# adobe-research/DiffusionHandles

Hardware: AMD Instinct MI355X
Metric: guided-denoise steps/sec at 512x512 (SD2-depth) (higher is better)
Workload: dtype f16; 1 GPU; single 512x512 edit per GPU, SD2-depth (865.9M params, seeded random weights), guided phase: 3 x (fwd + energy + bwd-to-latent) + CFG fwd (B=2) + DDIM step; resolution=512, edits_per_gpu=1, correspondences=24906, parallelism=independent edits, one process per GPU, no collectives

## Files before the change

### diffusionhandles_amd/_lib.py

```python
import ctypes
import os

import torch

_HERE = os.path.dirname(os.path.abspath(__file__))
LIB_PATH = os.environ.get("DIFFHANDLES_LIB") or os.path.join(_HERE, "libdiffhandles_hip.so")
_LIB = None

c_p = ctypes.c_void_p
c_i = ctypes.c_int
c_f = ctypes.c_float
c_d = ctypes.c_double
c_sz = ctypes.c_size_t


class UNetConfig(ctypes.Structure):
    _fields_ = [("in_channels", c_i), ("out_channels", c_i), ("n_levels", c_i),
                ("block_out_channels", c_i * 4), ("layers_per_block", c_i), ("heads", c_i * 4),
                ("cross_attention_dim", c_i), ("norm_groups", c_i), ("sample_size", c_i),
                ("text_len", c_i), ("max_batch", c_i), ("dtype", c_i), ("max_diff_batch", c_i)]


class VAEConfig(ctypes.Structure):
    _fields_ = [("latent_channels", c_i), ("out_channels", c_i), ("block_out_channels", c_i * 4),
# ... 88 lines not shown
    "dh_latent_update": (c_i, [c_p, c_p, c_p, c_f, c_f, c_i, c_p]),
    "dh_adam_step": (c_i, [c_p, c_p, c_p, c_p, c_f, c_f, c_f, c_f, c_i, c_i, c_p]),
    "dh_mse_fwd_bwd": (c_i, [c_p, c_p, c_i, c_p, c_p, c_p]),
    "dh_latent_update_strided": (c_i, [c_p, c_p, c_p, c_i, c_i, c_f, c_f, c_i, c_p]),
    "dh_pack_sample": (c_i, [c_p, c_p, c_i, c_i, c_p, c_i, c_i, c_i, c_i, c_p]),
    "dh_unet_io_ptr": (c_i, [c_p, c_i, c_i, ctypes.POINTER(c_p), ctypes.POINTER(c_sz)]),
    "dh_mse_cotangent": (c_i, [c_p, c_p, c_i, c_f, c_f, c_p, c_p, c_p, c_p]),
    "dh_adam_step_scaled": (c_i, [c_p, c_p, c_p, c_p, c_p, c_f, c_f, c_f, c_f, c_i, c_i, c_p]),
    "dh_mse_cotangent_batch": (c_i, [c_p, c_p, c_i, c_i, c_f, c_f, c_d, c_p, c_p, c_p, c_p, c_p, c_p]),
    "dh_adam_step_scaled_batch": (c_i, [c_p, c_p, c_p, c_p, c_p, c_p, c_f, c_f, c_f, c_f, c_i, c_i, c_i, c_p]),
    "dh_latent_update_guarded": (c_i, [c_p, c_p, c_p, c_i, c_i, c_f, c_i, c_i, c_p, c_i, c_i, c_p, c_p, c_i, c_i, c_p]),
    "dh_ddim_cfg_step_flagged": (c_i, [c_p, c_p, c_p, c_p, c_f, c_f, c_f, c_i, c_i, c_p, c_i, c_i, c_p]),
}

c_l = ctypes.c_long
DEBUG_SIGNATURES = {
    "dh_dbg_gemm": (c_i, [c_i, c_p, c_l, c_p, c_i, c_i, c_i, c_i, c_i, c_i, c_i, c_i, c_i, c_i, c_i, c_p, c_p, c_i, c_i,
                          c_p, c_l, c_p, c_l, c_i, c_p, c_sz, c_p]),
    "dh_dbg_gemm_groupnorm": (c_i, [c_i, c_p, c_l, c_p, c_i, c_i, c_i, c_i, c_i, c_i, c_i, c_p, c_p, c_p, c_sz, c_i, c_i, c_p, c_p, c_f, c_i,
                                    c_p, c_p, c_p, ctypes.POINTER(c_i), c_p]),
    "dh_dbg_gemm_groupnorm_bwd": (c_i, [c_i, c_p, c_l, c_p, c_i, c_i, c_i, c_i, c_i, c_i, c_i, c_p, c_p, c_sz, c_i, c_i, c_p, c_p, c_p, c_p, c_i,
                                        c_p, c_p, ctypes.POINTER(c_i), c_p]),
    "dh_dbg_gemm_groupnorm_res": (c_i, [c_i, c_p, c_l, c_p, c_i, c_i, c_i, c_i, c_i, c_i, c_i, c_p, c_p, c_l, c_p, c_p, c_sz, c_i, c_i, c_p, c_p,
                                    c_f, c_i, c_p, c_p, c_p, ctypes.POINTER(c_i), c_p]),
    "dh_dbg_gemm_groupnorm_bwd_res": (c_i, [c_i, c_p, c_l, c_p, c_i, c_i, c_i, c_i, c_i, c_i, c_i, c_p, c_l, c_p, c_p, c_sz, c_i, c_i, c_p, c_p, c_p,
                                        c_p, c_i, c_p, c_p, ctypes.POINTER(c_i), c_p]),
    "dh_dbg_concat_groupnorm": (c_i, [c_i, c_p, c_i, c_p, c_i, c_p, c_i, c_i, c_i, c_p, c_p, c_f, c_i, c_p, c_p, c_p, c_p]),
    "dh_dbg_gemm_last_tile": (c_i, [ctypes.POINTER(c_i)]),
    "dh_dbg_unet_concat_ops": (c_i, [ctypes.POINTER(UNetConfig), ctypes.POINTER(c_i), c_i, ctypes.POINTER(c_i)]),
    "dh_dbg_gemm_lnfold": (c_i, [c_i, c_p, c_l, c_p, c_i, c_i, c_i, c_p, c_p, c_p, c_f, c_p, c_l, c_p]),
    "dh_dbg_gemm_glu": (c_i, [c_i, c_i, c_p, c_l, c_p, c_i, c_i, c_i, c_p, c_p, c_p, c_p, c_p, c_p]),
    "dh_dbg_gemm_glub_split": (c_i, [c_i, c_p, c_l, c_p, c_i, c_i, c_i, c_i, c_p, c_l, c_i, c_p, c_p, ctypes.POINTER(c_i), c_p]),
    "dh_dbg_unet_ff_fold": (c_i, [c_p, c_i, ctypes.POINTER(c_i), ctypes.POINTER(c_i), c_p, c_p, c_p]),
    "dh_dbg_gemm_family": (c_i, [c_i]),
    "dh_dbg_gemm_stage": (c_i, [c_i]),
    "dh_dbg_gemm_xattn": (c_i, [c_i, c_p, c_l, c_p, c_i, c_i, c_i, c_p, c_p, c_p, c_p, c_f, c_p, c_p, c_p, c_l, c_p, c_p, c_i, c_i, c_i,
                                ctypes.POINTER(c_i), c_p]),
    "dh_dbg_gemm_xattn_dq": (c_i, [c_i, c_p, c_l, c_p, c_i, c_i, c_i, c_p, c_p, c_p, c_p, c_l, c_p, c_p, c_p, c_i, c_i, ctypes.POINTER(c_i), c_p]),
    "dh_dbg_gemm_xattn_carried": (c_i, [ctypes.POINTER(c_i), ctypes.POINTER(ctypes.c_longlong)]),
    "dh_dbg_gemm_pp_variant": (c_i, [c_i, c_p]),
    "dh_dbg_gemm_pp_ablate": (c_i, [c_i]),
    "dh_dbg_gemm_pp_persist": (c_i, [c_i]),
    "dh_dbg_gemm_pp_glu": (c_i, [c_i]),
    "dh_dbg_gemm_pp_plan": (c_i, [c_i, c_i, c_i, c_i, c_i, c_i, c_sz, ctypes.POINTER(c_i), ctypes.POINTER(c_i), ctypes.POINTER(c_i)]),
    "dh_dbg_touch_tiled": (c_i, [c_sz, c_p]),
    "dh_dbg_groupnorm": (c_i, [c_i, c_p, c_p, c_p, c_p, c_p, c_p, c_p, c_p, c_i, c_i, c_i, c_i, c_f, c_i, c_i, c_p]),
    "dh_dbg_layernorm": (c_i, [c_i, c_p, c_p, c_p, c_p, c_p, c_p, c_p, c_p, c_i, c_i, c_f, c_p]),
    "dh_dbg_geglu": (c_i, [c_i, c_p, c_p, c_p, c_p, c_i, c_i, c_p]),
    "dh_dbg_attention": (c_i, [c_i, c_p, c_l, c_p, c_p, c_l, c_p, c_l, c_p, c_p, c_p, c_p, c_p, c_p, c_i, c_i, c_i, c_i, c_p]),
    "dh_dbg_attention_bwd_pair": (c_i, [c_i, c_p, c_l, c_p, c_p, c_l, c_p, c_l, c_p, c_p, c_p, c_p, c_p, c_p, c_i, c_i, c_i, c_i, c_p, c_p]),
    "dh_dbg_pool2x2": (c_i, [c_i, c_p, c_p, c_i, c_i, c_i, c_i, c_i, c_p]),
    "dh_dbg_ellipse_offsets": (c_i, [c_i, ctypes.POINTER(ctypes.c_int32), c_i, ctypes.POINTER(c_i)]),
    "dh_dbg_lane_ops": (c_i, [c_p, c_p, c_p, c_p]),
}


def lib():
    global _LIB
    if _LIB is None:
        if not os.path.exists(LIB_PATH):
            raise RuntimeError(
                f"native HIP library not found at {LIB_PATH}; build it with "
                "`python -c 'import __graft_entry__ as g; g.build()'` (there is no CPU fallback)")
        handle = ctypes.CDLL(LIB_PATH)
        missing = []
        for name, (res, args) in list(SIGNATURES.items()) + list(DEBUG_SIGNATURES.items()):
# ... 39 lines not shown
```

### diffusionhandles_amd/csrc/unet_engine.cpp

```cpp
#include <stdlib.h>

#include <algorithm>
#include <map>
#include <numeric>
#include <vector>

#include "unet_kernels.h"

namespace dh {

enum OpType { OP_CONV_IN, OP_CONV_OUT, OP_GEMM, OP_GN, OP_LN, OP_ATTN, OP_GEGLU, OP_CONCAT, OP_TIMESTEP, OP_T2F };
enum ParamKind { PK_F32, PK_MAT };

struct Ten {
  size_t off = 0, goff = 0;
  size_t off_fo = 0;
  int rows = 0, C = 0;
  int ld = 0;
  int view = -1, col = 0;
  bool req_grad = true;
  bool persistent = false;
};

struct Wt {
  size_t fwd_off = 0, bwd_off = 0;
  int N = 0, K = 0, taps = 1;
  bool has_bwd = true, f32 = false;
  int glu_F = 0;
};

struct ParamInfo {
  std::string name;
  int ndim = 0;
  int64_t shape[4] = {0, 0, 0, 0};
  int kind = PK_F32;
  size_t f32_off = 0;
  int wt = -1;
  int row_off = 0;
  int glu_F = 0;
};

struct Op {
  int type = OP_GEMM;
// ... 15 lines not shown
  int xattn_bwd_op = -1;
};

struct FfFold {
  int wt_po = -1, wt_ffo = -1, wt = -1;
  long b_po = -1, b_ffo = -1, bias = -1;
};

}

using namespace dh;

struct dh_unet {
  dh_unet_config cfg;
  int dtype = DH_DTYPE_F16;
  std::vector<Ten> tens;
  std::vector<Wt> wts;
  std::vector<ParamInfo> params;
  std::vector<Op> ops;
  std::vector<FfFold> ffolds;
  std::map<std::string, int> pindex;
  size_t w16_elems = 0, pf_elems = 0, act_elems = 0, grad_elems = 0, f32_elems = 0;
  size_t fo_elems = 0;
  size_t partial_elems = 0, scratch_elems = 0, small_elems = 0;
  unsigned short *w16 = nullptr, *act = nullptr, *grad = nullptr, *scratch = nullptr;
  float *pf = nullptr, *f32a = nullptr, *partial = nullptr, *small = nullptr;
  int t_text = -1, t_kv = -1, t_conv_in_out = -1, t_final = -1, act_ids[3] = {-1, -1, -1};
  int act_op_end[3] = {0, 0, 0};
  int first_cross_op = 0;
  int saved_ops = 0;
  int temb_ops = 0, temb_rows = 0;
  float temb_t = 0.f;
  hipStream_t temb_stream = nullptr;
  uint64_t text_key = 0, kv_key = 0;
  int kv_rows = 0;
  hipStream_t kv_stream = nullptr;
  long temb_f32_off = -1;
  int temb_total = 0, kv_total = 0;
  float *in_sample = nullptr, *in_text = nullptr, *io_eps = nullptr, *out_dsample = nullptr, *out_dtext = nullptr, *t_dev = nullptr;
  std::map<uint64_t, hipGraphExec_t> graphs;
  std::map<uint64_t, double> graph_flops;
  bool use_graphs = true;
  long ones_off = -1, zeros_off = -1;
  bool fold_dirty = true;
  bool owns_weights = true;
  int n_shared = 0;
  int saved_batch = 0;
  const float* saved_sample = nullptr;
  std::vector<char> gready;
  double flops_fwd = 0, flops_bwd = 0;
  int64_t launches = 0;

  bool fo_mode = false;
  unsigned short* aptr(int t, int B_unused = 0) { return act + (fo_mode && !tens[t].persistent ? tens[t].off_fo : tens[t].off); }
  std::vector<int> galias;
  unsigned short* gptr(int t) {
    while (galias[t] != t) t = galias[t];
    return grad + tens[t].goff;
  }
};

namespace {

struct Builder {
  dh_unet& u;
  int maxB, maxBd;
// ... 51 lines not shown

  int gn(int x, const std::string& pre, float eps, bool silu) {
    const Ten tx = u.tens[x];
    Op o;
    o.type = OP_GN; o.in0 = x; o.out = tensor(tx.rows, tx.C);
    o.gamma_off = param_f32(pre + ".weight", tx.C);
    o.beta_off = param_f32(pre + ".bias", tx.C);
    o.eps = eps; o.silu = silu; o.groups = u.cfg.norm_groups;
    o.stats_off = f32_slot((size_t)maxB * o.groups * 2);
    u.ops.push_back(o);
    return o.out;
  }
  int ln(int x, const std::string& pre) {
    const Ten tx = u.tens[x];
    Op o;
    o.type = OP_LN; o.in0 = x; o.out = tensor(tx.rows, tx.C);
    o.gamma_off = param_f32(pre + ".weight", tx.C);
    o.beta_off = param_f32(pre + ".bias", tx.C);
    o.eps = 1e-5f;
    o.stats_off = f32_slot((size_t)maxB * tx.rows * 2);
    u.ops.push_back(o);
    return o.out;
  }
  int conv3(int x, const std::string& pre, int Cout, int Hs, int stride, int up, long temb_off, int res) {
    const Ten& tx = u.tens[x];
    const int Cin = tx.C;
    const int Hv = Hs << up, Ho = stride == 2 ? Hv / 2 : Hv;
    Op o;
    o.type = OP_GEMM; o.mode = A_CONV3; o.in0 = x; o.res = res;
    o.Hin = Hs; o.Win = Hs; o.Cin = Cin; o.Hout = Ho; o.Wout = Ho; o.stride = stride; o.up = up;
    o.wt = weight(Cout, 9 * Cin, 9);
    bind_mat(pre + ".weight", o.wt, Cout, 0, Cin, 9);
    o.bias_off = param_f32(pre + ".bias", Cout);
    if (temb_off >= 0) { o.rowvec_off = u.temb_f32_off + temb_off; o.rowvec_ld = u.temb_total; }
    o.out = tensor(Ho * Ho, Cout);
    u.ops.push_back(o);
    return o.out;
  }
  int linear_w(int x, int wt, long bias_off, int res, int in_col = 0, int in_cols = 0, bool silu = false,
               bool req_grad = true) {
    const Ten tx = u.tens[x];
    Op o;
    o.type = OP_GEMM; o.mode = A_DENSE; o.in0 = x; o.res = res; o.wt = wt; o.bias_off = bias_off;
    o.in_col = in_col; o.in_cols = in_cols ? in_cols : tx.C; o.act_silu = silu;
    o.out = tensor(tx.rows, u.wts[wt].N, req_grad);
    u.ops.push_back(o);
    return o.out;
  }
  int linear(int x, const std::string& pre, int N, bool bias, int res, bool as_conv1x1 = false) {
    const int K = u.tens[x].C;
    const int wt = weight(N, K);
    if (as_conv1x1) bind_conv1x1(pre + ".weight", wt, N, K); else bind_mat(pre + ".weight", wt, N, 0, K, 1);
    const long b = bias ? param_f32(pre + ".bias", N) : -1;
    return linear_w(x, wt, b, res);
  }
  int concat(int a, int b) {
    Op o;
    o.type = OP_CONCAT; o.in0 = a; o.in1 = b;
    o.out = tensor(u.tens[a].rows, u.tens[a].C + u.tens[b].C);
    u.ops.push_back(o);
    return o.out;
  }

  void fold_ln_into_last_gemm() {
    const int gi = (int)u.ops.size() - 1, li = gi - 1;
    Op& g = u.ops[gi];
    Op& l = u.ops[li];
// ... 96 lines not shown
  }
  temb_total += 2 * c.block_out_channels[L - 1];
  kv_total += 2 * c.block_out_channels[L - 1];
  for (int i = 0; i < L; ++i) {
    const int ch = c.block_out_channels[L - 1 - i];
    temb_total += (n + 1) * ch;
    if (i > 0) kv_total += (n + 1) * 2 * ch;
  }
}

static void layout_tensors(dh_unet& u);
static size_t ff_fold_scratch(int C);

int build(dh_unet& u) {
  const dh_unet_config& c = u.cfg;
  Builder b(u);
  const int L = c.n_levels, n = c.layers_per_block, S = c.sample_size;
  const int* ch = c.block_out_channels;
  const int temb_dim = ch[0] * 4;
  count_fused(c, u.temb_total, u.kv_total);

  int t_sin = b.tensor(1, ch[0], false);
  { Op o; o.type = OP_TIMESTEP; o.out = t_sin; u.ops.push_back(o); }
  const int w1 = b.weight(temb_dim, ch[0], 1, false);
  b.bind_mat("time_embedding.linear_1.weight", w1, temb_dim, 0, ch[0], 1);
  int e1 = b.linear_w(t_sin, w1, b.param_f32("time_embedding.linear_1.bias", temb_dim), -1, 0, 0, true, false);
  const int w2 = b.weight(temb_dim, temb_dim, 1, false);
  b.bind_mat("time_embedding.linear_2.weight", w2, temb_dim, 0, temb_dim, 1);
  int e2 = b.linear_w(e1, w2, b.param_f32("time_embedding.linear_2.bias", temb_dim), -1, 0, 0, true, false);
  b.wt_temb = b.weight(u.temb_total, temb_dim, 1, false);
  b.temb_bias_off = u.pf_elems;
  u.pf_elems += align_up((size_t)u.temb_total, 64);
  int t_temb = b.linear_w(e2, b.wt_temb, (long)b.temb_bias_off, -1, 0, 0, false, false);
  u.temb_f32_off = (long)b.f32_slot((size_t)c.max_batch * u.temb_total);
  { Op o; o.type = OP_T2F; o.in0 = t_temb; u.ops.push_back(o); }
  u.temb_ops = (int)u.ops.size();

  u.t_text = b.tensor(c.text_len, c.cross_attention_dim, true);
  b.wt_kv = b.weight(u.kv_total, c.cross_attention_dim);
  u.t_kv = b.linear_w(u.t_text, b.wt_kv, -1, -1);

  { Op o;
    o.type = OP_CONV_IN;
    o.wt = b.weight(ch[0], 9 * c.in_channels, 9, true, true);
    b.bind_mat("conv_in.weight", o.wt, ch[0], 0, c.in_channels, 9);
    o.bias_off = b.param_f32("conv_in.bias", ch[0]);
    o.Hin = S; o.Cin = c.in_channels;
    o.out = b.tensor(S * S, ch[0]);
    u.t_conv_in_out = o.out;
    u.ops.push_back(o); }
  int x = u.t_conv_in_out;
  std::vector<int> skips{x};
  int H = S;
  for (int i = 0; i < L; ++i) {
    const std::string pre = "down_blocks." + std::to_string(i);
    const bool attn = i < L - 1, down = i < L - 1;
    for (int j = 0; j < n; ++j) {
      x = b.resnet(x, pre + ".resnets." + std::to_string(j), ch[i], H);
      if (attn) x = b.transformer(x, pre + ".attentions." + std::to_string(j), c.heads[i], H);
      skips.push_back(x);
    }
    if (down) {
      x = b.conv3(x, pre + ".downsamplers.0.conv", ch[i], H, 2, 0, -1, -1);
      H /= 2;
      skips.push_back(x);
    }
  }
// ... 309 lines not shown
    dh_unet_destroy(u);
    return DH_ERR_HIP;
  };
  hipError_t e;
  if (parent) {
    if (u->w16_elems != parent->w16_elems || u->pf_elems != parent->pf_elems) {
      set_error("internal: shared engine lays its parameters out differently");
      delete u;
      return DH_ERR_STATE;
    }
    u->owns_weights = false;
    u->w16 = parent->w16; u->pf = parent->pf;
    u->fold_dirty = false;
  } else {
    if ((e = hipMalloc((void**)&u->w16, u->w16_elems * 2 + 256)) != hipSuccess) return fail(e, "hipMalloc weights");
    if ((e = hipMalloc((void**)&u->pf, u->pf_elems * 4 + 256)) != hipSuccess) return fail(e, "hipMalloc f32 params");
  }
  if ((e = hipMalloc((void**)&u->act, u->act_elems * 2 + 256)) != hipSuccess) return fail(e, "hipMalloc activations");
  if ((e = hipMalloc((void**)&u->grad, u->grad_elems * 2 + 256)) != hipSuccess) return fail(e, "hipMalloc gradients");
  if ((e = hipMalloc((void**)&u->f32a, u->f32_elems * 4 + 256)) != hipSuccess) return fail(e, "hipMalloc f32 arena");
  if ((e = hipMalloc((void**)&u->partial, u->partial_elems * 4)) != hipSuccess) return fail(e, "hipMalloc split-K");
  if ((e = hipMalloc((void**)&u->scratch, u->scratch_elems * 2)) != hipSuccess) return fail(e, "hipMalloc scratch");
  if ((e = hipMalloc((void**)&u->small, u->small_elems * 4)) != hipSuccess) return fail(e, "hipMalloc small");
  {
    const dh_unet_config& c = u->cfg;
    const size_t ns = (size_t)c.max_batch * c.sample_size * c.sample_size;
    const size_t nt = (size_t)c.max_batch * c.text_len * c.cross_attention_dim;
    if ((e = hipMalloc((void**)&u->in_sample, ns * c.in_channels * 4)) != hipSuccess) return fail(e, "hipMalloc staging");
    if ((e = hipMalloc((void**)&u->out_dsample, ns * c.in_channels * 4)) != hipSuccess) return fail(e, "hipMalloc staging");
    if ((e = hipMalloc((void**)&u->io_eps, ns * c.out_channels * 4)) != hipSuccess) return fail(e, "hipMalloc staging");
    if ((e = hipMalloc((void**)&u->in_text, nt * 4)) != hipSuccess) return fail(e, "hipMalloc staging");
    if ((e = hipMalloc((void**)&u->out_dtext, nt * 4)) != hipSuccess) return fail(e, "hipMalloc staging");
    if ((e = hipMalloc((void**)&u->t_dev, 64)) != hipSuccess) return fail(e, "hipMalloc staging");
    u->use_graphs = !(getenv("DH_GRAPH") && atoi(getenv("DH_GRAPH")) == 0);
  }
  if (!parent) {
    (void)hipMemset(u->w16, 0, u->w16_elems * 2);
    (void)hipMemset(u->pf, 0, u->pf_elems * 4);
  }
  u->gready.assign(u->tens.size(), 0);
  u->galias.resize(u->tens.size());
  std::iota(u->galias.begin(), u->galias.end(), 0);
  *out = u;
  return DH_OK;
}

extern "C" int dh_unet_create_shared(dh_unet* parent, int max_batch, void* stream, dh_unet** out) {
  DH_REQUIRE(parent && out, "null pointer");
  DH_REQUIRE(parent->owns_weights, "share from the engine that owns the weights");
  dh_unet_config cfg = parent->cfg;
  if (max_batch > 0 && max_batch != cfg.max_batch) { cfg.max_batch = max_batch; cfg.max_diff_batch = 0; }
  DH_REQUIRE(cfg.max_batch < 4096 && (long)cfg.max_batch * cfg.sample_size * cfg.sample_size < (1L << 21), "bad max_batch");
  if (parent->fold_dirty) {
    fold_layernorms(parent, (hipStream_t)stream);
    DH_CHECK_HIP(hipStreamSynchronize((hipStream_t)stream));
  }
  int rc = create_engine(&cfg, parent, out);
  if (rc == DH_OK) ++parent->n_shared;
  return rc;
}

extern "C" void dh_unet_destroy(dh_unet* u) {
  if (!u) return;
  if (u->owns_weights) { (void)hipFree(u->w16); (void)hipFree(u->pf); }
  (void)hipFree(u->act); (void)hipFree(u->grad);
  (void)hipFree(u->f32a); (void)hipFree(u->partial); (void)hipFree(u->scratch); (void)hipFree(u->small);
  (void)hipFree(u->in_sample); (void)hipFree(u->in_text); (void)hipFree(u->io_eps); (void)hipFree(u->out_dsample);
  (void)hipFree(u->out_dtext); (void)hipFree(u->t_dev);
  for (auto& kv : u->graphs) (void)hipGraphExecDestroy(kv.second);
  delete u;
}

extern "C" int dh_unet_num_params(const dh_unet* u) { return u ? (int)u->params.size() : 0; }

extern "C" int dh_unet_param_info(const dh_unet* u, int i, const char** name, int* ndim, int64_t* shape4) {
  DH_REQUIRE(u && i >= 0 && i < (int)u->params.size() && name && ndim && shape4, "bad arguments");
  const ParamInfo& p = u->params[i];
  *name = p.name.c_str();
  *ndim = p.ndim;
  for (int k = 0; k < 4; ++k) shape4[k] = p.shape[k];
  return DH_OK;
}

extern "C" int dh_unet_load_param(dh_unet* u, int i, const float* src, void* stream) {
  DH_REQUIRE(u && src && i >= 0 && i < (int)u->params.size(), "bad arguments");
  if (!u->owns_weights || u->n_shared > 0) {
    set_error("dh_unet_load_param: the weights are shared (dh_unet_create_shared): load every parameter before sharing");
    return DH_ERR_STATE;
  }
  u->temb_rows = 0; u->fold_dirty = true; u->kv_key = 0;
  hipStream_t st = (hipStream_t)stream;
  const ParamInfo& p = u->params[i];
  if (p.kind == PK_F32) {
    if (p.glu_F) {
      hipLaunchKernelGGL(k_load_glu_bias, dim3(cdiv((int)p.shape[0], 256)), dim3(256), 0, st, src, u->pf + p.f32_off, p.glu_F);
      DH_LAUNCH_CHECK();
      return DH_OK;
    }
    DH_CHECK_HIP(hipMemcpyAsync(u->pf + p.f32_off, src, (size_t)p.shape[0] * 4, hipMemcpyDeviceToDevice, st));
    return DH_OK;
  }
  const Wt& w = u->wts[p.wt];
  const int N = (int)p.shape[0], C = (int)p.shape[1], taps = w.taps;
  const size_t total = (size_t)N * C * taps;
  const unsigned nb = (unsigned)((total + 255) / 256);
  const long fwd_ld = w.K;
  const long bwd_ld = (long)taps * w.N;
  if (w.f32) {
    float* f = u->pf + w.fwd_off;
    float* b = w.has_bwd ? u->pf + w.bwd_off : nullptr;
    hipLaunchKernelGGL((k_load_weight<float, false>), dim3(nb), dim3(256), 0, st, src, N, C, taps, f, fwd_ld, (long)p.row_off,
                       b, bwd_ld, (long)p.row_off, w.N);
  } else if (u->dtype == DH_DTYPE_F16) {
    f16* f = (f16*)(u->w16 + w.fwd_off);
    f16* b = w.has_bwd ? (f16*)(u->w16 + w.bwd_off) : nullptr;
    hipLaunchKernelGGL((k_load_weight<f16, true>), dim3(nb), dim3(256), 0, st, src, N, C, taps, f, fwd_ld, (long)p.row_off, b,
                       bwd_ld, (long)p.row_off, w.N, 1.f, w.glu_F);
  } else {
    bf16* f = (bf16*)(u->w16 + w.fwd_off);
    bf16* b = w.has_bwd ? (bf16*)(u->w16 + w.bwd_off) : nullptr;
    hipLaunchKernelGGL((k_load_weight<bf16, true>), dim3(nb), dim3(256), 0, st, src, N, C, taps, f, fwd_ld, (long)p.row_off, b,
                       bwd_ld, (long)p.row_off, w.N, 1.f, w.glu_F);
  }
  DH_LAUNCH_CHECK();
  return DH_OK;
}

extern "C" size_t dh_unet_weight_bytes(const dh_unet* u) { return u && u->owns_weights ? u->w16_elems * 2 + u->pf_elems * 4 : 0; }
extern "C" size_t dh_unet_workspace_bytes(const dh_unet* u) {
  return u ? (u->act_elems + u->grad_elems + u->scratch_elems) * 2 + (u->f32_elems + u->partial_elems + u->small_elems) * 4 : 0;
}

static void fill_gemm(dh_unet* u, const Op& o, int B, GemmArgs& g) {
  const Wt& w = u->wts[o.wt];
  const Ten& ti = u->tens[o.in0];
  const Ten& to = u->tens[o.out];
  g.A = u->aptr(o.in0) + o.in_col; g.lda = ti.ld;
  g.W = u->w16 + w.fwd_off;
  g.M = B * to.rows; g.N = w.N; g.K = w.K;
  g.mode = o.mode; g.Hin = o.Hin; g.Win = o.Win; g.Cin = o.Cin; g.Hout = o.Hout; g.Wout = o.Wout;
  g.stride = o.stride; g.up = o.up;
  g.bias = o.bias_off >= 0 ? u->pf + o.bias_off : nullptr;
  if (o.rowvec_off >= 0) { g.rowvec = u->f32a + o.rowvec_off; g.rowvec_ld = o.rowvec_ld; g.rows_per_batch = to.rows; }
  if (o.res >= 0) { g.R = u->aptr(o.res); g.ldr = u->tens[o.res].ld; }
  g.C = u->aptr(o.out); g.ldc = to.ld;
  g.act_silu = o.act_silu;
  g.partial = u->partial; g.partial_elems = u->partial_elems;
  if (o.ln_fold >= 0) {
    const Op& l = u->ops[o.ln_fold];
    if (use_ln_fold(u, B)) {
      g.A = u->aptr(l.in0); g.lda = u->tens[l.in0].ld;
      g.bias = nullptr;
      g.ln_s = u->pf + o.ln_s_off; g.ln_t = u->pf + o.ln_t_off; g.ln_stats = u->f32a + l.stats_off; g.ln_eps = l.eps;
    } else {
      g.bias = u->pf + o.ln_t_off;
    }
  }
}

static void forward_ops(dh_unet* u, int B, int n_ops, int first_op, bool kv_hit, bool save, hipStream_t st) {
  const int dt = u->dtype;
  const dh_unet_config& c = u->cfg;
  u->flops_fwd = 0;
  int gn_have = 0;
  int xa_have = 0;
  if (!kv_hit) launch_f32_to_t(dt, u->in_text, u->aptr(u->t_text), (size_t)B * c.text_len * c.cross_attention_dim, st);
  for (int oi = first_op; oi < n_ops; ++oi) {
    const Op& o = u->ops[oi];
    if (kv_hit && oi == u->temb_ops) continue;
    switch (o.type) {
      case OP_TIMESTEP:
        launch_timestep_embedding(dt, u->t_dev, c.block_out_channels[0], B, u->aptr(o.out), st);
        break;
      case OP_T2F:
        launch_t_to_f32(dt, u->aptr(o.in0), u->f32a + u->temb_f32_off, (size_t)B * u->temb_total, 0, st);
        break;
      case OP_CONV_IN: {
        const Wt& w = u->wts[o.wt];
        launch_conv_small_fwd(dt, u->in_sample, 1, u->pf + w.fwd_off, u->pf + o.bias_off, u->aptr(o.out), 0, B, o.Hin, o.Hin,
                              o.Cin, w.N, st);
        u->flops_fwd += 2.0 * B * o.Hin * o.Hin * w.N * w.K;
        break;
      }
      case OP_CONV_OUT: {
        const Wt& w = u->wts[o.wt];
        launch_conv_small_fwd(dt, u->aptr(o.in0), 0, u->pf + w.fwd_off, u->pf + o.bias_off, u->io_eps, 1, B, o.Hin, o.Hin,
                              o.Cin, w.N, st);
        u->flops_fwd += 2.0 * B * o.Hin * o.Hin * w.N * w.K;
        break;
      }
      case OP_GEMM: {
        GemmArgs g;
        fill_gemm(u, o, B, g);
        gn_have = 0;
        if (o.gn_next >= 0 && oi + 1 < n_ops) {
          const Ten& to = u->tens[o.out];
          g.gn_part = u->small; g.gn_HW = to.rows; g.gn_G = u->ops[o.gn_next].groups; g.gn_done = &gn_have;
        }
        if (o.glu_op >= 0 && o.glu_op < n_ops) {
          const Op& ge = u->ops[o.glu_op];
          g.glu_y = u->aptr(ge.out); g.glu_ldy = u->tens[ge.out].ld;
          if (!save) g.C = nullptr;
// ... 84 lines not shown
    DH_CHECK_HIP(hipStreamBeginCapture(st, hipStreamCaptureModeThreadLocal));
    body();
    DH_CHECK_HIP(hipStreamEndCapture(st, &graph));
    hipGraphExec_t exec = nullptr;
    DH_CHECK_HIP(hipGraphInstantiate(&exec, graph, nullptr, nullptr, 0));
    (void)hipGraphDestroy(graph);
    u->graphs[key] = exec;
    u->graph_flops[key] = *flops_slot;
    it = u->graphs.find(key);
  }
  *flops_slot = u->graph_flops[key];
  DH_CHECK_HIP(hipGraphLaunch(it->second, st));
  return DH_OK;
}

extern "C" int dh_unet_forward(dh_unet* u, const float* sample, float timestep, const float* text, int batch,
                               int save_for_backward, float* eps_out, void* const* act_out, void* stream) {
  DH_REQUIRE(u && sample && text, "null pointer");
  DH_REQUIRE(batch >= 1 && batch <= u->cfg.max_batch, "batch exceeds max_batch");
  DH_REQUIRE(!save_for_backward || batch <= u->cfg.max_diff_batch, "a forward saved for a backward pass exceeds max_diff_batch");
  hipStream_t st = (hipStream_t)stream;
  const int B = batch;
  const dh_unet_config& c = u->cfg;
  const size_t ns = (size_t)B * c.sample_size * c.sample_size;
  if (sample != u->in_sample) DH_CHECK_HIP(hipMemcpyAsync(u->in_sample, sample, ns * c.in_channels * 4, hipMemcpyDeviceToDevice, st));
  int n_ops = (int)u->ops.size();
  if (!eps_out) {
    n_ops = 0;
    for (int i = 0; i < 3; ++i)
      if (act_out && act_out[i]) n_ops = std::max(n_ops, u->act_op_end[i]);
    DH_REQUIRE(n_ops > 0, "nothing requested: eps_out and every act_out are null");
  }
  if (u->fold_dirty) fold_layernorms(u, st);
  const bool temb_hit = u->temb_rows >= B && u->temb_t == timestep && u->temb_stream == st;
  const bool kv_hit = u->text_key != 0 && u->text_key == u->kv_key && u->kv_rows == B && u->kv_stream == st;
  const int first_op = temb_hit ? u->temb_ops : 0;
  if (!kv_hit && text != u->in_text)
    DH_CHECK_HIP(hipMemcpyAsync(u->in_text, text, (size_t)B * c.text_len * c.cross_attention_dim * 4, hipMemcpyDeviceToDevice, st));
  if (!temb_hit) launch_set_scalar(u->t_dev, timestep, st);
  const bool save = save_for_backward != 0;
  u->fo_mode = !save;
  int rc = run_graphed(u, graph_key_fwd(B, n_ops, temb_hit, kv_hit, save), st, &u->flops_fwd,
                       [&]() { forward_ops(u, B, n_ops, first_op, kv_hit, save, st); });
  u->fo_mode = false;
  if (rc != DH_OK) { u->temb_rows = 0; u->kv_key = 0; return rc; }
  if (!temb_hit) { u->temb_t = timestep; u->temb_rows = B; u->temb_stream = st; }
  if (!kv_hit) { u->kv_key = u->text_key; u->kv_rows = B; u->kv_stream = st; }
  if (eps_out && eps_out != u->io_eps)
    DH_CHECK_HIP(hipMemcpyAsync(eps_out, u->io_eps, ns * c.out_channels * 4, hipMemcpyDeviceToDevice, st));
  if (act_out) {
    for (int i = 0; i < 3; ++i)
      if (act_out[i]) {
        DH_REQUIRE(u->act_op_end[i] <= n_ops, "activation requested beyond the truncated tape");
        const Ten& t = u->tens[u->act_ids[i]];
        if (act_out[i] != (void*)u->aptr(u->act_ids[i]))
          DH_CHECK_HIP(hipMemcpyAsync(act_out[i], u->aptr(u->act_ids[i]), (size_t)B * t.rows * t.C * 2,
                                      hipMemcpyDeviceToDevice, st));
      }
  }
  u->saved_batch = save_for_backward ? B : 0;
  u->saved_ops = n_ops;
  DH_LAUNCH_CHECK();
  return DH_OK;
}

namespace {
struct Bwd {
  dh_unet* u;
  int B, dt;
  hipStream_t st;
  bool need_text;
  void add_into(int t, const unsigned short* src, long lds_, int cols, int col_off = 0) {
    const Ten& tt = u->tens[t];
    launch_copy_cols(dt, src, lds_, u->gptr(t) + col_off, tt.C, B * tt.rows, cols, u->gready[t] ? 1 : 0, st);
  }
};
}

static void backward_ops(dh_unet* u, int B, unsigned act_mask, bool has_eps, bool want_sample, bool want_text,
// ... 271 lines not shown

extern "C" int dh_unet_io_ptr(dh_unet* u, int which, int index, void** ptr, size_t* bytes) {
  DH_REQUIRE(u && ptr, "null pointer");
  const dh_unet_config& c = u->cfg;
  const size_t ns = (size_t)c.max_batch * c.sample_size * c.sample_size;
  const size_t nt = (size_t)c.max_batch * c.text_len * c.cross_attention_dim;
  size_t n = 0;
  switch (which) {
    case DH_IO_SAMPLE: *ptr = u->in_sample; n = ns * c.in_channels * 4; break;
    case DH_IO_TEXT: *ptr = u->in_text; n = nt * 4; break;
    case DH_IO_EPS: *ptr = u->io_eps; n = ns * c.out_channels * 4; break;
    case DH_IO_DSAMPLE: *ptr = u->out_dsample; n = ns * c.in_channels * 4; break;
    case DH_IO_DTEXT: *ptr = u->out_dtext; n = nt * 4; break;
    case DH_IO_ACT:
    case DH_IO_ACT_GRAD: {
      DH_REQUIRE(index >= 0 && index < 3 && u->act_ids[index] >= 0, "activation index out of range");
      const Ten& t = u->tens[u->act_ids[index]];
      *ptr = which == DH_IO_ACT ? (void*)(u->act + t.off) : (void*)(u->grad + t.goff);
      n = (size_t)(which == DH_IO_ACT ? c.max_batch : c.max_diff_batch) * t.rows * t.C * 2;
      break;
    }
    default: DH_REQUIRE(false, "unknown buffer");
  }
  if (bytes) *bytes = n;
  return DH_OK;
}

extern "C" int dh_unet_set_text_key(dh_unet* u, unsigned long long key) {
  DH_REQUIRE(u, "null engine");
  u->text_key = key;
  return DH_OK;
}

extern "C" int dh_unet_stats(const dh_unet* u, double* flops_fwd, double* flops_bwd, int64_t* launches) {
  DH_REQUIRE(u, "null engine");
  if (flops_fwd) *flops_fwd = u->flops_fwd;
  if (flops_bwd) *flops_bwd = u->flops_bwd;
  if (launches) *launches = (int64_t)u->ops.size();
  return DH_OK;
}

extern "C" int dh_dbg_unet_concat_ops(const dh_unet_config* cfg, int* out, int cap, int* n_out) {
  DH_REQUIRE(cfg && n_out && (out || cap == 0), "null pointer");
  dh_unet u;
  u.cfg = *cfg;
  const int rc = build(u);
  if (rc != DH_OK) return rc;
  int n = 0;
  for (size_t i = 0; i < u.ops.size(); ++i) {
    const Op& o = u.ops[i];
    if (o.type != OP_CONCAT) continue;
    const Ten &a = u.tens[o.in0], &b = u.tens[o.in1], &t = u.tens[o.out];
    const int G = o.gn_next >= 0 ? u.ops[o.gn_next].groups : 0;
    const bool fused = o.gn_next >= 0 && i + 1 < u.ops.size() && a.C % 8 == 0 && b.C % 8 == 0 && t.C % G == 0 &&
                       (GN_GB * (t.C / G)) % 8 == 0 && GN_GB * (t.C / G) <= 2048;
    if (n < cap) {
      int* e = out + 5 * n;
      e[0] = a.C; e[1] = b.C; e[2] = t.rows; e[3] = G; e[4] = fused ? 1 : 0;
    }
    ++n;
  }
  *n_out = n;
  return DH_OK;
}

extern "C" int dh_dbg_unet_ff_fold(dh_unet* u, int i, int* n_folds, int* C, void* w, float* bias, void* stream) {
// ... 17 lines not shown
```

### diffusionhandles_amd/unet.py

```python
import ctypes
import math
from types import SimpleNamespace

import torch

from . import _lib

SD2_DEPTH = dict(in_channels=5, out_channels=4, block_out_channels=(320, 640, 1280, 1280),
                 layers_per_block=2, heads=(5, 10, 20, 20), cross_attention_dim=1024,
                 norm_groups=32, sample_size=64, text_len=77)


class HipUNet:
    def __init__(self, cfg=None, dtype=torch.float16, max_batch=2, device=None, max_diff_batch=None):
        _lib.require_gpu()
        self.cfg = dict(SD2_DEPTH if cfg is None else cfg)
        self.cfg.setdefault("text_len", 77)
        self.dtype = dtype
        self.max_batch = int(max_batch)
        self.max_diff_batch = self.max_batch if not max_diff_batch else max(1, min(int(max_diff_batch), self.max_batch))
        self.device = torch.device("cuda", torch.cuda.current_device()) if device is None else torch.device(device)
        c = _lib.UNetConfig()
        c.in_channels, c.out_channels, c.n_levels = self.cfg["in_channels"], self.cfg["out_channels"], 4
        for i in range(4):
# ... 163 lines not shown
            p, nb = ctypes.c_void_p(), ctypes.c_size_t()
            _lib.check(self._L.dh_unet_io_ptr(self._h, code, index, ctypes.byref(p), ctypes.byref(nb)), "dh_unet_io_ptr")
            s, mb = self.sample_size, self.max_batch
            if which in ("act", "act_grad"):
                shape = (mb if which == "act" else self.max_diff_batch,) + self.act_shapes[index]
                t = torch.as_tensor(HipUNet._Raw(p.value, shape, "<i2"), device=self.device).view(self.dtype)
            else:
                shape = {"sample": (mb, s, s, self.cfg["in_channels"]), "dsample": (mb, s, s, self.cfg["in_channels"]),
                         "eps": (mb, s, s, self.cfg["out_channels"]),
                         "text": (mb, self.cfg["text_len"], self.cfg["cross_attention_dim"]),
                         "dtext": (mb, self.cfg["text_len"], self.cfg["cross_attention_dim"])}[which]
                t = torch.as_tensor(HipUNet._Raw(p.value, shape, "<f4"), device=self.device)
            assert t.data_ptr() == p.value and t.numel() * t.element_size() == nb.value
            self._views[key] = t
        return self._views[key]

    def stage_sample(self, latent_nhwc, depth_nhwc, batch):
        dst = self.io_view("sample")
        cl = latent_nhwc.shape[-1]
        cd = depth_nhwc.shape[-1] if depth_nhwc is not None else 0
        if cl + cd != self.cfg["in_channels"] or batch > self.max_batch:
            raise ValueError("stage_sample: channels / batch do not match the engine")
        pixels = self.sample_size * self.sample_size
        _lib.check(self._L.dh_pack_sample(_lib.ptr(dst), _lib.ptr(latent_nhwc), latent_nhwc.shape[0], cl, _lib.ptr(depth_nhwc),
                                          depth_nhwc.shape[0] if depth_nhwc is not None else 1, cd, batch, pixels,
                                          _lib.stream_ptr()), "dh_pack_sample")
        return dst[:batch]

    def stats(self):
        f, b, n = ctypes.c_double(), ctypes.c_double(), ctypes.c_int64()
        _lib.check(self._L.dh_unet_stats(self._h, ctypes.byref(f), ctypes.byref(b), ctypes.byref(n)))
        return dict(flops_fwd=f.value, flops_bwd=b.value, ops=n.value)

    def __call__(self, sample, timestep, encoder_hidden_states, cross_attention_kwargs=None, return_dict=True):
        x = sample.detach().to(self.device, torch.float32).permute(0, 2, 3, 1).contiguous()
        txt = encoder_hidden_states.detach().to(self.device, torch.float32).contiguous()
        t = float(timestep.item()) if isinstance(timestep, torch.Tensor) else float(timestep)
        eps, acts = self.forward(x, t, txt, save_for_backward=False, want_acts=not return_dict)
        eps = eps.permute(0, 3, 1, 2)
        if return_dict:
            return {"sample": eps}
        a = [t_.permute(0, 3, 1, 2) for t_ in acts]
        return (eps, None, None, None, a[0], a[1], a[2])
```

Measured before the change: 36.37 steps/s.

## Compute time embedding once per batch and cache it per timestep in a device table

The timestep-embedding chain now always runs at batch 1, and the conv ops broadcast one embedding row through a zero row stride instead of reading one row per batch entry. Each computed embedding is stored in a 64-slot device table keyed by timestep, so a later call at the same timestep copies the row back instead of rerunning the MLP chain. Within one denoise step every forward already shares a timestep, and the old single-entry cache already hit there, so the main saving is the smaller chain on the B=2 CFG pass when it misses. It adds a device-to-device copy on each miss and assumes all batch entries share one timestep.

```diff
diff --git a/diffusionhandles_amd/_lib.py b/diffusionhandles_amd/_lib.py
--- a/diffusionhandles_amd/_lib.py
+++ b/diffusionhandles_amd/_lib.py
@@ -144,6 +144,7 @@
     "dh_dbg_gemm_glu": (c_i, [c_i, c_i, c_p, c_l, c_p, c_i, c_i, c_i, c_p, c_p, c_p, c_p, c_p, c_p]),
     "dh_dbg_gemm_glub_split": (c_i, [c_i, c_p, c_l, c_p, c_i, c_i, c_i, c_i, c_p, c_l, c_i, c_p, c_p, ctypes.POINTER(c_i), c_p]),
     "dh_dbg_unet_ff_fold": (c_i, [c_p, c_i, ctypes.POINTER(c_i), ctypes.POINTER(c_i), c_p, c_p, c_p]),
+    "dh_dbg_unet_temb_stats": (c_i, [c_p, ctypes.POINTER(ctypes.c_int64), ctypes.POINTER(ctypes.c_int64), ctypes.POINTER(c_i)]),
     "dh_dbg_gemm_family": (c_i, [c_i]),
     "dh_dbg_gemm_stage": (c_i, [c_i]),
     "dh_dbg_gemm_xattn": (c_i, [c_i, c_p, c_l, c_p, c_i, c_i, c_i, c_p, c_p, c_p, c_p, c_f, c_p, c_p, c_p, c_l, c_p, c_p, c_i, c_i, c_i,
diff --git a/diffusionhandles_amd/csrc/unet_engine.cpp b/diffusionhandles_amd/csrc/unet_engine.cpp
--- a/diffusionhandles_amd/csrc/unet_engine.cpp
+++ b/diffusionhandles_amd/csrc/unet_engine.cpp
@@ -9,6 +9,7 @@
 
 namespace dh {
 
+constexpr int TEMB_SLOTS = 64;
 enum OpType { OP_CONV_IN, OP_CONV_OUT, OP_GEMM, OP_GN, OP_LN, OP_ATTN, OP_GEGLU, OP_CONCAT, OP_TIMESTEP, OP_T2F };
 enum ParamKind { PK_F32, PK_MAT };
 
@@ -90,6 +91,11 @@
   int temb_ops = 0, temb_rows = 0;
   float temb_t = 0.f;
   hipStream_t temb_stream = nullptr;
+  float* temb_table = nullptr;
+  std::vector<float> temb_keys;
+  int temb_next = 0;
+  int64_t temb_chain_runs = 0, temb_table_copies = 0;
+  void temb_clear() { temb_rows = 0; temb_keys.clear(); temb_next = 0; }
   uint64_t text_key = 0, kv_key = 0;
   int kv_rows = 0;
   hipStream_t kv_stream = nullptr;
@@ -207,7 +213,7 @@
     o.wt = weight(Cout, 9 * Cin, 9);
     bind_mat(pre + ".weight", o.wt, Cout, 0, Cin, 9);
     o.bias_off = param_f32(pre + ".bias", Cout);
-    if (temb_off >= 0) { o.rowvec_off = u.temb_f32_off + temb_off; o.rowvec_ld = u.temb_total; }
+    if (temb_off >= 0) { o.rowvec_off = u.temb_f32_off + temb_off; o.rowvec_ld = 0; }
     o.out = tensor(Ho * Ho, Cout);
     u.ops.push_back(o);
     return o.out;
@@ -370,7 +376,7 @@
   b.temb_bias_off = u.pf_elems;
   u.pf_elems += align_up((size_t)u.temb_total, 64);
   int t_temb = b.linear_w(e2, b.wt_temb, (long)b.temb_bias_off, -1, 0, 0, false, false);
-  u.temb_f32_off = (long)b.f32_slot((size_t)c.max_batch * u.temb_total);
+  u.temb_f32_off = (long)b.f32_slot((size_t)u.temb_total);
   { Op o; o.type = OP_T2F; o.in0 = t_temb; u.ops.push_back(o); }
   u.temb_ops = (int)u.ops.size();
 
@@ -746,6 +752,7 @@
     if ((e = hipMalloc((void**)&u->in_text, nt * 4)) != hipSuccess) return fail(e, "hipMalloc staging");
     if ((e = hipMalloc((void**)&u->out_dtext, nt * 4)) != hipSuccess) return fail(e, "hipMalloc staging");
     if ((e = hipMalloc((void**)&u->t_dev, 64)) != hipSuccess) return fail(e, "hipMalloc staging");
+    if ((e = hipMalloc((void**)&u->temb_table, (size_t)TEMB_SLOTS * u->temb_total * 4)) != hipSuccess) return fail(e, "hipMalloc time-embedding table");
     u->use_graphs = !(getenv("DH_GRAPH") && atoi(getenv("DH_GRAPH")) == 0);
   }
   if (!parent) {
@@ -780,7 +787,7 @@
   (void)hipFree(u->act); (void)hipFree(u->grad);
   (void)hipFree(u->f32a); (void)hipFree(u->partial); (void)hipFree(u->scratch); (void)hipFree(u->small);
   (void)hipFree(u->in_sample); (void)hipFree(u->in_text); (void)hipFree(u->io_eps); (void)hipFree(u->out_dsample);
-  (void)hipFree(u->out_dtext); (void)hipFree(u->t_dev);
+  (void)hipFree(u->out_dtext); (void)hipFree(u->t_dev); (void)hipFree(u->temb_table);
   for (auto& kv : u->graphs) (void)hipGraphExecDestroy(kv.second);
   delete u;
 }
@@ -802,7 +809,7 @@
     set_error("dh_unet_load_param: the weights are shared (dh_unet_create_shared): load every parameter before sharing");
     return DH_ERR_STATE;
   }
-  u->temb_rows = 0; u->fold_dirty = true; u->kv_key = 0;
+  u->temb_clear(); u->fold_dirty = true; u->kv_key = 0;
   hipStream_t st = (hipStream_t)stream;
   const ParamInfo& p = u->params[i];
   if (p.kind == PK_F32) {
@@ -842,7 +849,7 @@
 
 extern "C" size_t dh_unet_weight_bytes(const dh_unet* u) { return u && u->owns_weights ? u->w16_elems * 2 + u->pf_elems * 4 : 0; }
 extern "C" size_t dh_unet_workspace_bytes(const dh_unet* u) {
-  return u ? (u->act_elems + u->grad_elems + u->scratch_elems) * 2 + (u->f32_elems + u->partial_elems + u->small_elems) * 4 : 0;
+  return u ? (u->act_elems + u->grad_elems + u->scratch_elems) * 2 + (u->f32_elems + u->partial_elems + u->small_elems + (size_t)TEMB_SLOTS * u->temb_total) * 4 : 0;
 }
 
 static void fill_gemm(dh_unet* u, const Op& o, int B, GemmArgs& g) {
@@ -872,16 +879,17 @@
   }
 }
 
-static void forward_ops(dh_unet* u, int B, int n_ops, int first_op, bool kv_hit, bool save, hipStream_t st) {
+static void forward_ops(dh_unet* u, int Bpass, int n_ops, int first_op, bool kv_hit, bool save, hipStream_t st) {
   const int dt = u->dtype;
   const dh_unet_config& c = u->cfg;
   u->flops_fwd = 0;
   int gn_have = 0;
   int xa_have = 0;
-  if (!kv_hit) launch_f32_to_t(dt, u->in_text, u->aptr(u->t_text), (size_t)B * c.text_len * c.cross_attention_dim, st);
+  if (!kv_hit) launch_f32_to_t(dt, u->in_text, u->aptr(u->t_text), (size_t)Bpass * c.text_len * c.cross_attention_dim, st);
   for (int oi = first_op; oi < n_ops; ++oi) {
     const Op& o = u->ops[oi];
     if (kv_hit && oi == u->temb_ops) continue;
+    const int B = oi < u->temb_ops ? 1 : Bpass;
     switch (o.type) {
       case OP_TIMESTEP:
         launch_timestep_embedding(dt, u->t_dev, c.block_out_channels[0], B, u->aptr(o.out), st);
@@ -1032,7 +1040,19 @@
     DH_REQUIRE(n_ops > 0, "nothing requested: eps_out and every act_out are null");
   }
   if (u->fold_dirty) fold_layernorms(u, st);
-  const bool temb_hit = u->temb_rows >= B && u->temb_t == timestep && u->temb_stream == st;
+  if (u->temb_stream != st) u->temb_clear();
+  bool temb_hit = u->temb_rows != 0 && u->temb_t == timestep;
+  if (!temb_hit) {
+    for (size_t i = 0; i < u->temb_keys.size() && !temb_hit; ++i)
+      if (u->temb_keys[i] == timestep) {
+        DH_CHECK_HIP(hipMemcpyAsync(u->f32a + u->temb_f32_off, u->temb_table + i * (size_t)u->temb_total, (size_t)u->temb_total * 4,
+                                    hipMemcpyDeviceToDevice, st));
+        ++u->temb_table_copies;
+        u->temb_t = timestep; u->temb_rows = 1;
+        temb_hit = true;
+      }
+  }
+  const bool temb_ran = !temb_hit;
   const bool kv_hit = u->text_key != 0 && u->text_key == u->kv_key && u->kv_rows == B && u->kv_stream == st;
   const int first_op = temb_hit ? u->temb_ops : 0;
   if (!kv_hit && text != u->in_text)
@@ -1043,8 +1063,16 @@
   int rc = run_graphed(u, graph_key_fwd(B, n_ops, temb_hit, kv_hit, save), st, &u->flops_fwd,
                        [&]() { forward_ops(u, B, n_ops, first_op, kv_hit, save, st); });
   u->fo_mode = false;
-  if (rc != DH_OK) { u->temb_rows = 0; u->kv_key = 0; return rc; }
-  if (!temb_hit) { u->temb_t = timestep; u->temb_rows = B; u->temb_stream = st; }
+  if (rc != DH_OK) { u->temb_clear(); u->kv_key = 0; return rc; }
+  if (temb_ran) {
+    u->temb_t = timestep; u->temb_rows = 1; u->temb_stream = st;
+    ++u->temb_chain_runs;
+    const size_t row = (size_t)u->temb_next;
+    u->temb_next = (u->temb_next + 1) % TEMB_SLOTS;
+    if (row == u->temb_keys.size()) u->temb_keys.push_back(timestep); else u->temb_keys[row] = timestep;
+    DH_CHECK_HIP(hipMemcpyAsync(u->temb_table + row * (size_t)u->temb_total, u->f32a + u->temb_f32_off, (size_t)u->temb_total * 4,
+                                hipMemcpyDeviceToDevice, st));
+  }
   if (!kv_hit) { u->kv_key = u->text_key; u->kv_rows = B; u->kv_stream = st; }
   if (eps_out && eps_out != u->io_eps)
     DH_CHECK_HIP(hipMemcpyAsync(eps_out, u->io_eps, ns * c.out_channels * 4, hipMemcpyDeviceToDevice, st));
@@ -1382,6 +1410,14 @@
   return DH_OK;
 }
 
+extern "C" int dh_dbg_unet_temb_stats(const dh_unet* u, int64_t* chain_runs, int64_t* table_copies, int* filed) {
+  DH_REQUIRE(u, "null engine");
+  if (chain_runs) *chain_runs = u->temb_chain_runs;
+  if (table_copies) *table_copies = u->temb_table_copies;
+  if (filed) *filed = (int)u->temb_keys.size();
+  return DH_OK;
+}
+
 extern "C" int dh_unet_stats(const dh_unet* u, double* flops_fwd, double* flops_bwd, int64_t* launches) {
   DH_REQUIRE(u, "null engine");
   if (flops_fwd) *flops_fwd = u->flops_fwd;
diff --git a/diffusionhandles_amd/unet.py b/diffusionhandles_amd/unet.py
--- a/diffusionhandles_amd/unet.py
+++ b/diffusionhandles_amd/unet.py
@@ -219,6 +219,11 @@
         _lib.check(self._L.dh_unet_stats(self._h, ctypes.byref(f), ctypes.byref(b), ctypes.byref(n)))
         return dict(flops_fwd=f.value, flops_bwd=b.value, ops=n.value)
 
+    def temb_stats(self):
+        r, c, n = ctypes.c_int64(), ctypes.c_int64(), ctypes.c_int()
+        _lib.check(self._L.dh_dbg_unet_temb_stats(self._h, ctypes.byref(r), ctypes.byref(c), ctypes.byref(n)))
+        return dict(chain_runs=r.value, table_copies=c.value, filed=n.value)
+
     def __call__(self, sample, timestep, encoder_hidden_states, cross_attention_kwargs=None, return_dict=True):
         x = sample.detach().to(self.device, torch.float32).permute(0, 2, 3, 1).contiguous()
         txt = encoder_hidden_states.detach().to(self.device, torch.float32).contiguous()
```

After: 36.46 steps/s, median of 6. About the same (+0.2%).
